# KingOfTheAce2/video-restoration-pipeline-framewright

Hardware: AMD Instinct MI355X
Metric: frames/sec Real-ESRGAN x4 1080p (RRDBNet-x4plus, 1920x1080 -> 7680x4320) (higher is better)
Workload: dtype f16; 1 GPU; RealESRGAN_x4plus x4, 1920x1080 uint8 BGR frames resident in HBM -> 7680x4320 uint8 BGR in HBM, seeded synthetic weights, 43 frames per GPU

## Files before the change

include/framewright_hip.h:

```cpp
#ifndef FRAMEWRIGHT_HIP_H
#define FRAMEWRIGHT_HIP_H

#include <stddef.h>
#include <stdint.h>

#ifdef __cplusplus
extern "C" {
#endif

#define FW_OK 0
#define FW_ERR_INVALID 1
#define FW_ERR_OOM 2
#define FW_ERR_HIP 3
#define FW_ERR_INTERNAL 4

#define FW_HOST 0
#define FW_DEVICE 1

#define FW_DTYPE_BF16 0
#define FW_DTYPE_F16 1

typedef struct fw_rrdbnet fw_rrdbnet;
typedef struct fw_nafnet fw_nafnet;

// ... 35 lines not shown
                    int width, const void* packed_weight, const float* bias, int cout_tiles, int act_lrelu,
                    int upsample2x, const float* res1, float s1, const float* res2, float s2, void* out,
                    int out_cstride, long out_plane_stride, int out_coff, float* out_f32, void* stream);

int fw_conv3x3_nhwc_ex(int dtype, const void* x, int in_cstride, long in_plane_stride, int cin_chunks, int height,
                       int width, const void* packed_weight, const float* bias, int cout_tiles, int act_lrelu,
                       int upsample2x, const float* res1, float s1, const float* res2, float s2, const float* chan_scale,
                       int post_act, int f32_cstride, int f32_coff, void* out, int out_cstride, long out_plane_stride,
                       int out_coff, float* out_f32, void* stream);


int fw_u8_to_nhwc(int dtype, const uint8_t* in_bgr, int height, int width, void* out, int out_cstride, void* stream);

int fw_pixel_shuffle_add_u8(const float* conv, int conv_cstride, const uint8_t* in_bgr, int height, int width, int scale,
                            uint8_t* out_bgr, float* out_rgb_f32, void* stream);

int fw_conv3x3_pair_nhwc(int dtype, const void* x, int in_cstride, long in_plane_stride, int in_chunks, int height,
                         int width, const void* packed_weight_a, const float* bias_a, const void* packed_weight_b,
                         const float* bias_b, void* out_a, void* out_b, int out_cstride, void* stream);

size_t fw_pack_conv_up2x_phase(int dtype, const float* weight, uint16_t* dst);
int fw_conv_up2x_phase_nhwc(int dtype, const void* x, int in_cstride, long in_plane_stride, int height, int width,
                            const void* packed_weight, const float* bias, int act_lrelu, void* out, int out_cstride,
                            long out_plane_stride, void* stream);

size_t fw_pack_conv3x3_wino(int dtype, const float* weight, int cout, int cin, int cin_chunks, uint16_t* dst);
int fw_conv3x3_split_nhwc(int dtype, int winograd, const void* x, int in_cstride, long in_plane_stride, int cin_chunks, int height,
                          int width, const void* packed_weight, const float* bias, float s1, float in_id_scale, int n_id,
                          const long* chunk_off, const float* id_scale, int post_act, void* out, void* out_lo, int out_cstride,
                          long out_plane_stride, int out_coff, void* stream);
int fw_conv3x3_wino_nhwc(int dtype, const void* x, int in_cstride, long in_plane_stride, int cin_chunks, int height, int width,
                         const void* packed_weight, const float* bias, int act_lrelu, void* out, int out_cstride,
                         long out_plane_stride, int out_coff, void* stream);
int fw_conv3x3_wino_check_fields(int* codes, int n);


int fw_nafnet_create(int device_id, int width, int middle_blk_num, const int* enc_blk_nums, const int* dec_blk_nums,
                     int num_levels, int dtype, fw_nafnet** out);

int fw_nafnet_set_tensor(fw_nafnet* net, const char* key, const float* data, size_t numel);
int fw_nafnet_finalize(fw_nafnet* net);

int fw_nafnet_denoise_u8(fw_nafnet* net, const uint8_t* in_bgr, int in_loc, int height, int width, uint8_t* out_bgr,
                         int out_loc, float* out_rgb_f32, void* stream);
double fw_nafnet_flops(const fw_nafnet* net, int height, int width);
int fw_nafnet_destroy(fw_nafnet* net);

#define FW_NAF_PATH_FRONT 1
#define FW_NAF_PATH_TAIL128 2
#define FW_NAF_PATH_TAIL64 4
#define FW_NAF_PATH_GEMM 8
#define FW_NAF_PATH_FUSE_LN 16
int fw_nafnet_run_block(fw_nafnet* net, const char* key, float* stream_f32, int height, int width, float* sca_out, void* stream);
int fw_nafnet_block_paths(fw_nafnet* net, const char* key, int* flags);
int fw_nafnet_run_resample(fw_nafnet* net, int level, int up, const float* src_f32, int height, int width, float* dst_f32, void* stream);
int fw_u8_to_nhwc_padded(int dtype, const uint8_t* in_bgr, int height, int width, int padded_height, int padded_width, void* out,
                         void* stream);


int fw_u8_crop(const uint8_t* src, int height, int width, int y0, int x0, int th, int tw, uint8_t* dst, void* stream);

int fw_tile_blend_accumulate(float* acc, float* wsum, int height, int width, const uint8_t* tile, int y0, int x0, int th,
                             int tw, int overlap, void* stream);

int fw_tile_blend_finish(const float* acc, const float* wsum, int height, int width, uint8_t* out, void* stream);

// ... 222 lines not shown
```

video-restoration-pipeline-framewright_amd/_lib.py:

```python
from __future__ import annotations

import ctypes as C
import threading
from pathlib import Path
from typing import Optional

PKG_DIR = Path(__file__).resolve().parent
LIB_PATH = PKG_DIR / "lib" / "libframewright_hip.so"

FW_OK, FW_ERR_INVALID, FW_ERR_OOM, FW_ERR_HIP, FW_ERR_INTERNAL = 0, 1, 2, 3, 4
FW_HOST, FW_DEVICE = 0, 1
FW_DTYPE_BF16, FW_DTYPE_F16 = 0, 1
FW_NAF_PATH_FRONT, FW_NAF_PATH_TAIL128, FW_NAF_PATH_TAIL64, FW_NAF_PATH_GEMM, FW_NAF_PATH_FUSE_LN = 1, 2, 4, 8, 16
DTYPES = {"bf16": FW_DTYPE_BF16, "bfloat16": FW_DTYPE_BF16, "f16": FW_DTYPE_F16, "fp16": FW_DTYPE_F16,
          "float16": FW_DTYPE_F16, "half": FW_DTYPE_F16}

EXPORTS = [
    "fw_last_error", "fw_abi_version", "fw_device_count",
    "fw_rrdbnet_create", "fw_rrdbnet_set_conv", "fw_rrdbnet_finalize", "fw_rrdbnet_upscale_u8", "fw_rrdbnet_upscale_u16",
    "fw_rrdbnet_workspace_bytes", "fw_rrdbnet_flops", "fw_rrdbnet_profile_enable", "fw_rrdbnet_profile_read",
    "fw_rrdbnet_destroy", "fw_pack_conv3x3", "fw_conv3x3_nhwc",
    "fw_nafnet_create", "fw_nafnet_set_tensor", "fw_nafnet_finalize", "fw_nafnet_denoise_u8", "fw_nafnet_flops",
    "fw_nafnet_destroy", "fw_nafnet_run_block", "fw_nafnet_block_paths", "fw_nafnet_run_resample", "fw_u8_to_nhwc_padded", "fw_u8_crop", "fw_tile_blend_accumulate", "fw_tile_blend_finish", "fw_temporal_average_u8",
    "fw_strength_blend_u8",
    "fw_conv3x3_nhwc_ex", "fw_conv3x3_pair_nhwc", "fw_pack_conv_up2x_phase", "fw_conv_up2x_phase_nhwc", "fw_u8_to_rgb_f32", "fw_resize_bilinear_f32", "fw_ifnet_build_x", "fw_unshuffle2_cast",
    "fw_depth_to_space4_f32", "fw_ifnet_accumulate", "fw_ifnet_blend", "fw_unsharp_mask_u8",
    "fw_ifnet_stage_input", "fw_ifnet_accumulate_d2s", "fw_ifnet_last_flow",
    "fw_ifnet_create", "fw_ifnet_set_tensor", "fw_ifnet_finalize", "fw_ifnet_interp_u8", "fw_ifnet_workspace_bytes", "fw_ifnet_flops",
    "fw_ifnet_destroy",
    "fw_aesrgan_create", "fw_aesrgan_set_tensor", "fw_aesrgan_finalize", "fw_aesrgan_forward_rgb", "fw_aesrgan_workspace_bytes", "fw_aesrgan_destroy",
    "fw_srvgg_create", "fw_srvgg_set_tensor", "fw_srvgg_finalize", "fw_srvgg_upscale_u8", "fw_srvgg_upscale_u16", "fw_resize_lanczos4_u16", "fw_srvgg_workspace_bytes", "fw_srvgg_flops",
    "fw_srvgg_destroy",
    "fw_restormer_create", "fw_restormer_set_tensor", "fw_restormer_finalize", "fw_restormer_denoise_u8",
    "fw_restormer_workspace_bytes", "fw_restormer_destroy", "fw_preserve_edges_scratch_bytes", "fw_preserve_edges_u8",
    "fw_u8_to_nhwc", "fw_pixel_shuffle_add_u8",
    "fw_layernorm_nhwc", "fw_pack_pointwise", "fw_pointwise_nhwc", "fw_dwconv3x3_nhwc", "fw_attn_workspace_floats",
    "fw_attn_matrix", "fw_attn_apply", "fw_attn_pack", "fw_attn_proj_pack", "fw_pixel_shuffle2_f32", "fw_copy_channels_f32", "fw_f32_to_planar", "fw_tap_post_u8",
    "fw_flow_accumulate_u8", "fw_flow_accumulate_finish_u8", "fw_resize_lanczos4_u8", "fw_resize_linear_u8", "fw_face_paste_u8", "fw_grain_addback_u8", "fw_attn_softmax_rows", "fw_pack_pointwise_transposed", "fw_attn_qk_scratch_elems", "fw_attn_matrix_mfma",
    "fw_pack_conv3x3_wino", "fw_conv3x3_split_nhwc", "fw_conv3x3_wino_nhwc", "fw_conv3x3_wino_check_fields",
    "fw_farneback_scratch_bytes", "fw_farneback_flow_u8", "fw_flow_stats_f32", "fw_flow_confidence_f32",
    "fw_nlmeans_scratch_bytes", "fw_nlmeans_u8", "fw_nlmeans_colored_u8", "fw_nlmeans_weight_table", "fw_nlmeans_lab_tables",
    "fw_frame_stats_u8", "fw_flow_accumulate_affine_u8", "fw_add_weighted_u8",
    "fw_bgr_to_lab_u8", "fw_lab_to_bgr_u8", "fw_lab_l_sums_u8", "fw_deflicker_lab_u8", "fw_gamma_lab_tables",
    "fw_scene_ssim_workspace_bytes", "fw_scene_ssim_u8", "fw_hist64x3_u8",
    "fw_pil_lanczos_taps", "fw_pil_thumb_workspace_bytes", "fw_pil_thumb_u8", "fw_dhash_pack_u8",
    "fw_lut3d_apply_u8", "fw_lut3d_apply_u16", "fw_table3_apply_u8",
    "fw_deinterlace_u8", "fw_deinterlace_batch_u8", "fw_interlace_stats_u8", "fw_frame_absdiff_sum_u8",
    "fw_vhs_gray_stats_u8", "fw_vhs_blend_rows_u8", "fw_vhs_rainbow_u8", "fw_vhs_box_gray_sums_u8", "fw_vhs_dropout_repair_u8",
    "fw_vhs_edge_counts_u8", "fw_vhs_chroma_samples_u8", "fw_vhs_chroma_shift_u8", "fw_vhs_column_sums_u8", "fw_vhs_jitter_shifts_u8",
    "fw_vhs_saturation_f64",
]


class FramewrightHipError(RuntimeError):

    def __init__(self, code: int, message: str):
        super().__init__(message)
        self.code = code


class FramewrightOutOfMemory(FramewrightHipError):
    """FW_ERR_OOM — message contains "memory" so reference restorer.py:1746 retries with a smaller tile."""


_lock = threading.Lock()
_lib: Optional[C.CDLL] = None


def _declare(lib: C.CDLL) -> None:
    vp, i32, f32, f64, sz = C.c_void_p, C.c_int, C.c_float, C.c_double, C.c_size_t
    lib.fw_last_error.restype = C.c_char_p
    lib.fw_last_error.argtypes = []
# ... 58 lines not shown
    lib.fw_tile_blend_finish.argtypes = [vp, vp, i32, i32, vp, vp]
    lib.fw_temporal_average_u8.restype = i32
    lib.fw_temporal_average_u8.argtypes = [C.POINTER(vp), C.POINTER(f32), i32, sz, vp, vp]
    lib.fw_strength_blend_u8.restype = i32
    lib.fw_strength_blend_u8.argtypes = [vp, vp, f64, sz, vp, vp]
    lib.fw_grain_addback_u8.restype = i32
    lib.fw_grain_addback_u8.argtypes = [vp, vp, i32, i32, f64, vp, vp, vp]
    lib.fw_resize_lanczos4_u8.restype = i32
    lib.fw_resize_lanczos4_u8.argtypes = [vp, i32, i32, i32, vp, i32, i32, vp]
    lib.fw_resize_linear_u8.restype = i32
    lib.fw_resize_linear_u8.argtypes = [vp, i32, i32, i32, vp, i32, i32, vp]
    lib.fw_face_paste_u8.restype = i32
    lib.fw_face_paste_u8.argtypes = [vp, i32, i32, i32, i32, i32, i32, vp, f64, vp]


def _declare_ifnet(lib: C.CDLL) -> None:
    vp, i32, f32, sz = C.c_void_p, C.c_int, C.c_float, C.c_size_t
    lib.fw_conv3x3_nhwc_ex.restype = i32
    lib.fw_conv3x3_nhwc_ex.argtypes = [i32, vp, i32, C.c_long, i32, i32, i32, vp, vp, i32, i32, i32, vp, f32, vp, f32, vp, i32,
                                       i32, i32, vp, i32, C.c_long, i32, vp, vp]
    lib.fw_pack_conv_up2x_phase.restype = sz
    lib.fw_pack_conv_up2x_phase.argtypes = [i32, vp, vp]
    lib.fw_conv_up2x_phase_nhwc.restype = i32
    lib.fw_conv_up2x_phase_nhwc.argtypes = [i32, vp, i32, C.c_long, i32, i32, vp, vp, i32, vp, i32, C.c_long, vp]
    lib.fw_pack_conv3x3_wino.restype = sz
    lib.fw_pack_conv3x3_wino.argtypes = [i32, vp, i32, i32, i32, vp]
    lib.fw_conv3x3_split_nhwc.restype = i32
    lib.fw_conv3x3_split_nhwc.argtypes = [i32, i32, vp, i32, C.c_long, i32, i32, i32, vp, vp, f32, f32, i32, C.POINTER(C.c_long),
                                          C.POINTER(f32), i32, vp, vp, i32, C.c_long, i32, vp]
    lib.fw_conv3x3_wino_nhwc.restype = i32
    lib.fw_conv3x3_wino_nhwc.argtypes = [i32, vp, i32, C.c_long, i32, i32, i32, vp, vp, i32, vp, i32, C.c_long, i32, vp]
    lib.fw_conv3x3_wino_check_fields.restype = i32
    lib.fw_conv3x3_wino_check_fields.argtypes = [C.POINTER(i32), i32]
    lib.fw_conv3x3_pair_nhwc.restype = i32
    lib.fw_conv3x3_pair_nhwc.argtypes = [i32, vp, i32, C.c_long, i32, i32, i32, vp, vp, vp, vp, vp, vp, i32, vp]
    lib.fw_u8_to_rgb_f32.restype = i32
    lib.fw_u8_to_rgb_f32.argtypes = [vp, i32, i32, i32, i32, vp, vp]
    lib.fw_resize_bilinear_f32.restype = i32
    lib.fw_resize_bilinear_f32.argtypes = [vp, i32, i32, i32, vp, i32, i32, i32, i32, f32, f32, vp]
    lib.fw_ifnet_build_x.restype = i32
    lib.fw_ifnet_build_x.argtypes = [vp, vp, vp, vp, i32, i32, f32, vp, vp]
    lib.fw_unshuffle2_cast.restype = i32
    lib.fw_unshuffle2_cast.argtypes = [i32, vp, i32, i32, i32, i32, i32, vp, i32, vp]
    lib.fw_depth_to_space4_f32.restype = i32
    lib.fw_depth_to_space4_f32.argtypes = [vp, i32, i32, i32, vp, vp]
    lib.fw_ifnet_accumulate.restype = i32
    lib.fw_ifnet_accumulate.argtypes = [vp, i32, i32, i32, i32, f32, vp, vp, i32, vp]
    lib.fw_ifnet_stage_input.restype = i32
    lib.fw_ifnet_stage_input.argtypes = [i32, vp, vp, vp, vp, i32, i32, f32, i32, vp, i32, vp]
    lib.fw_ifnet_accumulate_d2s.restype = i32
    lib.fw_ifnet_accumulate_d2s.argtypes = [vp, i32, i32, i32, i32, i32, f32, vp, vp, i32, vp]
    lib.fw_ifnet_last_flow.restype = i32
    lib.fw_ifnet_last_flow.argtypes = [vp, i32, i32, vp, vp, vp]
    lib.fw_ifnet_blend.restype = i32
    lib.fw_ifnet_blend.argtypes = [vp, vp, vp, vp, i32, i32, i32, i32, vp, vp, vp]
    lib.fw_aesrgan_create.restype = i32
    lib.fw_aesrgan_create.argtypes = [i32, i32, i32, i32, i32, C.POINTER(vp)]
    lib.fw_aesrgan_set_tensor.restype = i32
    lib.fw_aesrgan_set_tensor.argtypes = [vp, C.c_char_p, vp, sz]
    lib.fw_aesrgan_finalize.restype = i32
    lib.fw_aesrgan_finalize.argtypes = [vp]
    lib.fw_aesrgan_forward_rgb.restype = i32
    lib.fw_aesrgan_forward_rgb.argtypes = [vp, vp, i32, i32, vp, vp]
    lib.fw_aesrgan_workspace_bytes.restype = sz
    lib.fw_aesrgan_workspace_bytes.argtypes = [vp, i32, i32]
    lib.fw_aesrgan_destroy.restype = i32
# ... 297 lines not shown
```

video-restoration-pipeline-framewright_amd/csrc/fw_internal.h:

```cpp
#pragma once
#include <hip/hip_runtime.h>
#include <stdint.h>
#include <string.h>
#include <string>
#include <stdexcept>

namespace fw {

enum DType : int { DT_BF16 = 0, DT_F16 = 1 };

enum ConvEpilogue : int {
    EPI_STORE = 0,
    EPI_RESIDUAL = 1,
    EPI_IMAGE = 2,
    EPI_RESIDUAL_SPLIT = 3,
};

struct ConvParams {
    const void* in;
    int in_cstride;
    long in_pstride;
    int cin_chunks;
    int H, W;
    const void* wpk;
// ... 41 lines not shown
    const float* bias_a;
    const void* wpk_b;
    const float* bias_b;
    void* out_a;
    void* out_b;
    int out_cstride;
    const void* zeros;
    unsigned long long* stamps;
};
size_t pack_conv3x3_wino_weights(DType dt, const float* w, int cout, int cin, int cin_chunks, uint16_t* dst);
void launch_conv3x3_wino_split(const ConvParams& p, hipStream_t stream);
void launch_conv3x3_wino_store(const ConvParams& p, hipStream_t stream);
void check_conv3x3_wino(const ConvParams& p, bool split);
void launch_conv3x3_pair(DType dt, const ConvPairParams& p, hipStream_t stream);
const void* conv_zero_page();

struct ConvUpParams {
    const void* in;
    int in_cstride;
    long in_pstride;
    int H, W;
    const void* wpk;
    const float* bias;
    int act;
    void* out;
    int out_cstride;
    long out_pstride;
    const void* zeros;
};
void launch_conv_up2x_phase(DType dt, const ConvUpParams& p, hipStream_t stream);
size_t pack_conv_up2x_phase_weights(DType dt, const float* w, uint16_t* dst);
int conv_num_cus();

void launch_conv3x3(DType dt, int cout_tiles, ConvEpilogue epi, const ConvParams& p, hipStream_t stream);

size_t pack_conv3x3_weights(DType dt, const float* w, int cout, int cin, int cout_tiles, int cin_chunks,
                            uint16_t* dst);

void launch_u8_to_nhwc(DType dt, const uint8_t* in_bgr, int H, int W, void* out, int out_cstride,
                       int unshuffle, hipStream_t stream);
void launch_frame_to_nhwc(DType dt, const void* in_bgr, int bits, int H, int W, void* out, int out_cstride, int unshuffle,
                          hipStream_t stream);
void launch_pixel_shuffle_add(const float* conv, int cstride, const uint8_t* in_bgr, int H, int W, int scale, uint8_t* out_bgr,
                              float* out_rgb, hipStream_t stream);
void launch_pixel_shuffle_add_bits(const float* conv, int cstride, const void* in_bgr, int bits, int H, int W, int scale, void* out_bgr,
                                   float* out_rgb, hipStream_t stream);

enum PointwiseMode : int {
    PW_STORE = 0,
    PW_RESIDUAL = 1,
    PW_GATE = 2,
    PW_SHUFFLE_UP = 3,
};

struct PointwiseParams {
    const void* a;
    int a_f32;
    long lda;
    long M;
    int K;
    int gather2x2;
    int Win;
    int Cin;
    const float* a_scale;
    const float* ln_w;
    const float* ln_b;
// ... 235 lines not shown
```

video-restoration-pipeline-framewright_amd/csrc/rrdbnet.hip:

```cpp
#include <mutex>
#include <vector>
#include <memory>
#include <cstdio>
#include <cstdlib>
#include "engine_common.h"

namespace fw {

struct ConvLayer {
    int cout = 0, cin = 0, ct = 0, chunks = 0;
    void* d_w = nullptr;
    float* d_b = nullptr;
    void* d_wphase = nullptr;
    void* d_wwino = nullptr;
    bool set = false;
};

}

using namespace fw;

namespace fw {
std::string& last_error_ref() {
    thread_local std::string msg;
    return msg;
}
}

struct fw_rrdbnet {
    int device = 0;
    fw::StreamOrder order;
    int num_block = 0;
    int scale = 4;
    DType dt = DT_BF16;
    std::mutex mu;
    ConvLayer conv_first, conv_body, conv_up1, conv_up2, conv_hr, conv_last;
    std::vector<ConvLayer> body;
    DevBuf ws;
    int fuse_mask = 3;
    bool fuse_pairs = true;
    bool split_trunk = true;
    bool rrdb_lo = true;
    int abl_alias = 0;
    bool up_phase = true;
    int c5_wino = 1;
    bool hr_wino = false;
    int abl_rdb3 = 0;
    int graph_mode = 0;
    long graph_max_px = 512L * 512L;
    GraphCache graphs;
    bool warmed = false;
    bool profile = false;
    std::vector<hipEvent_t> ev_pool;
    size_t ev_used = 0;
    double prof_flops = 0;
    hipStream_t prof_stream = nullptr;
};

namespace {

size_t align_up(size_t v, size_t a) { return (v + a - 1) / a * a; }

void trunk_size(const fw_rrdbnet* n, int H, int W, int* Ht, int* Wt) {
    if (n->scale == 2) {
        *Ht = (H + 1) / 2;
        *Wt = (W + 1) / 2;
    } else {
        *Ht = H;
        *Wt = W;
    }
}

struct Plan {
    size_t in_u8, out_u8, in32, cat0, cat1, cat2, F, R, tA, tB, U1, U2, U3, total;
};

Plan make_plan(const fw_rrdbnet* n, int H, int W) {
    int Ht, Wt;
    trunk_size(n, H, W, &Ht, &Wt);
// ... 26 lines not shown
    p.U3 = take(px * 16 * 64 * 2);
    p.total = o;
    return p;
}

ConvLayer* find_layer(fw_rrdbnet* n, const std::string& key, int* want_cout, int* want_cin) {
    const int in_ch = n->scale == 2 ? 12 : 3;
    auto ret = [&](ConvLayer* l, int co, int ci) {
        *want_cout = co;
        *want_cin = ci;
        return l;
    };
    if (key == "conv_first") return ret(&n->conv_first, 64, in_ch);
    if (key == "conv_body") return ret(&n->conv_body, 64, 64);
    if (key == "conv_up1") return ret(&n->conv_up1, 64, 64);
    if (key == "conv_up2") return ret(&n->conv_up2, 64, 64);
    if (key == "conv_hr") return ret(&n->conv_hr, 64, 64);
    if (key == "conv_last") return ret(&n->conv_last, 3, 64);
    int b = -1, r = -1, c = -1;
    char tail = 0;
    if (sscanf(key.c_str(), "body.%d.rdb%d.conv%d%c", &b, &r, &c, &tail) == 3 && b >= 0 && b < n->num_block && r >= 1 &&
        r <= 3 && c >= 1 && c <= 5) {
        ConvLayer* l = &n->body[((size_t)b * 3 + (r - 1)) * 5 + (c - 1)];
        return ret(l, c == 5 ? 64 : 32, 64 + 32 * (c - 1));
    }
    return nullptr;
}

void free_layer(ConvLayer& l) {
    if (l.d_w) (void)hipFree(l.d_w);
    if (l.d_b) (void)hipFree(l.d_b);
    if (l.d_wphase) (void)hipFree(l.d_wphase);
    if (l.d_wwino) (void)hipFree(l.d_wwino);
    l.d_wphase = nullptr;
    l.d_wwino = nullptr;
    l.d_w = nullptr;
    l.d_b = nullptr;
    l.set = false;
}

double conv_flops(const ConvLayer& l, size_t pixels) { return 2.0 * 9.0 * l.cin * l.cout * (double)pixels; }

template <typename F>
void timed(fw_rrdbnet* n, hipStream_t st, double flops, F&& launch) {
    if (!n->profile) {
        launch();
        return;
    }
    if (n->ev_used + 2 > n->ev_pool.size()) {
        size_t old = n->ev_pool.size();
        n->ev_pool.resize(old + 1024);
        for (size_t i = old; i < n->ev_pool.size(); ++i) FW_HIP_CHECK(hipEventCreate(&n->ev_pool[i]));
    }
    FW_HIP_CHECK(hipEventRecord(n->ev_pool[n->ev_used++], st));
    launch();
    FW_HIP_CHECK(hipEventRecord(n->ev_pool[n->ev_used++], st));
    n->prof_flops += flops;
    n->prof_stream = st;
}

void run_conv(fw_rrdbnet* n, const ConvLayer& l, ConvEpilogue epi, ConvParams p, hipStream_t st) {
    p.cin_chunks = l.chunks;
    p.wpk = l.d_w;
    p.bias = l.d_b;
    timed(n, st, conv_flops(l, (size_t)p.H * p.W), [&] { launch_conv3x3(n->dt, l.ct, epi, p, st); });
}
// ... 154 lines not shown
        run_conv(n, n->conv_body, EPI_RESIDUAL, p, st);
        cur = (cur + 1) % ncat;
    }
    auto run_up = [&](const ConvLayer& l, const void* src, long src_pstride, int Hs, int Ws, void* dst, long dst_pstride) {
        if (n->up_phase && l.d_wphase) {
            ConvUpParams u{};
            u.in = src;
            u.in_cstride = 32;
            u.in_pstride = src_pstride;
            u.H = Hs;
            u.W = Ws;
            u.wpk = l.d_wphase;
            u.bias = l.d_b;
            u.act = 1;
            u.out = dst;
            u.out_cstride = 32;
            u.out_pstride = dst_pstride;
            timed(n, st, conv_flops(l, (size_t)4 * Hs * Ws), [&] { launch_conv_up2x_phase(n->dt, u, st); });
        } else {
            ConvParams p = base;
            p.H = 2 * Hs;
            p.W = 2 * Ws;
            p.in = src;
            p.in_pstride = src_pstride;
            p.upsample2x = 1;
            p.out = dst;
            p.out_pstride = dst_pstride;
            p.act = 1;
            run_conv(n, l, EPI_STORE, p, st);
        }
    };
    run_up(n->conv_up1, cat[cur], PL, Ht, Wt, U1, 4 * PL);
    run_up(n->conv_up2, U1, 4 * PL, 2 * Ht, 2 * Wt, U2, 16 * PL);
    {
        ConvParams p = base;
        p.H = 4 * Ht;
        p.W = 4 * Wt;
        p.in = U2;
        p.in_pstride = 16 * PL;
        p.out = U3;
        p.out_pstride = 16 * PL;
        p.act = 1;
        if (n->c5_wino && n->dt == DT_F16 && n->conv_hr.d_wwino && n->hr_wino) {
            p.cin_chunks = n->conv_hr.chunks;
            p.wpk = n->conv_hr.d_wwino;
            p.bias = n->conv_hr.d_b;
            timed(n, st, conv_flops(n->conv_hr, (size_t)p.H * p.W), [&] { launch_conv3x3_wino_store(p, st); });
        } else {
            run_conv(n, n->conv_hr, EPI_STORE, p, st);
        }
    }
    {
        ConvParams p = base;
        p.H = 4 * Ht;
        p.W = 4 * Wt;
        p.in = U3;
        p.in_pstride = 16 * PL;
        if (bits == 16)
            p.out_u16 = (uint16_t*)d_out;
        else
            p.out_u8 = (uint8_t*)d_out;
        p.out_rgb = d_rgb;
        p.img_H = n->scale * H;
        p.img_W = n->scale * W;
        run_conv(n, n->conv_last, EPI_IMAGE, p, st);
    }
}

}

extern "C" {

const char* fw_last_error(void) { return fw::last_error_ref().c_str(); }

int fw_abi_version(void) { return 4; }

int fw_device_count(void) {
    int n = 0;
    if (hipGetDeviceCount(&n) != hipSuccess) return 0;
    return n;
}

int fw_rrdbnet_create(int device_id, int num_block, int scale, int dtype, fw_rrdbnet** out) {
    if (!out) return fail(FW_ERR_INVALID, "fw_rrdbnet_create: out is NULL");
    *out = nullptr;
    if (num_block < 1 || num_block > 64) return fail(FW_ERR_INVALID, "fw_rrdbnet_create: num_block out of range");
    if (scale != 2 && scale != 4) return fail(FW_ERR_INVALID, "fw_rrdbnet_create: scale must be 2 or 4");
    if (dtype != FW_DTYPE_BF16 && dtype != FW_DTYPE_F16) return fail(FW_ERR_INVALID, "fw_rrdbnet_create: bad dtype");
    return guarded([&] {
        int ndev = 0;
        FW_HIP_CHECK(hipGetDeviceCount(&ndev));
        if (device_id < 0 || device_id >= ndev) throw Error(FW_ERR_INVALID, "fw_rrdbnet_create: no such device");
        auto n = std::make_unique<fw_rrdbnet>();
        n->device = device_id;
        n->num_block = num_block;
        n->scale = scale;
        n->dt = (DType)dtype;
        n->body.resize((size_t)num_block * 15);
        if (const char* e = getenv("FW_RRDB_FUSE_PAIRS")) n->fuse_pairs = atoi(e) != 0;
        if (const char* e = getenv("FW_RRDB_FUSE_MASK")) n->fuse_mask = atoi(e) & 3;
        if (const char* e = getenv("FW_RRDB_GRAPH")) n->graph_mode = atoi(e);
        if (const char* e = getenv("FW_RRDB_GRAPH_MAX_PX")) n->graph_max_px = atol(e);
        if (const char* e = getenv("FW_RRDB_SPLIT_TRUNK")) n->split_trunk = atoi(e) != 0;
        if (const char* e = getenv("FW_RRDB_LO")) n->rrdb_lo = atoi(e) != 0;
        if (const char* e = getenv("FW_RRDB_ABL_ALIAS")) n->abl_alias = atoi(e);
        if (const char* e = getenv("FW_RRDB_UP_PHASE")) n->up_phase = atoi(e) != 0;
        if (const char* e = getenv("FW_RRDB_ABL_RDB3")) n->abl_rdb3 = atoi(e);
        if (const char* e = getenv("FW_RRDB_C5_WINO")) n->c5_wino = atoi(e);
        if (const char* e = getenv("FW_RRDB_HR_WINO")) n->hr_wino = atoi(e) != 0;
        *out = n.release();
    });
}

int fw_rrdbnet_set_conv(fw_rrdbnet* n, const char* key, const float* weight, const float* bias, int cout, int cin) {
    if (!n || !key || !weight || !bias) return fail(FW_ERR_INVALID, "fw_rrdbnet_set_conv: NULL argument");
    return guarded([&] {
        std::lock_guard<std::mutex> lk(n->mu);
        int wco = 0, wci = 0;
        ConvLayer* l = find_layer(n, key, &wco, &wci);
        if (!l) throw Error(FW_ERR_INVALID, std::string("fw_rrdbnet_set_conv: unknown key '") + key + "'");
        if (cout != wco || cin != wci)
            throw Error(FW_ERR_INVALID, std::string("fw_rrdbnet_set_conv: shape mismatch for '") + key + "': got [" +
                                            std::to_string(cout) + "," + std::to_string(cin) + ",3,3], expected [" +
                                            std::to_string(wco) + "," + std::to_string(wci) + ",3,3]");
        DevGuard dg(n->device);
        free_layer(*l);
        l->cout = cout;
        l->cin = cin;
        l->ct = (cout + 31) / 32;
        l->chunks = (cin + 31) / 32;
        const size_t ne = pack_conv3x3_weights(n->dt, nullptr, cout, cin, l->ct, l->chunks, nullptr);
        std::vector<uint16_t> packed(ne);
        pack_conv3x3_weights(n->dt, weight, cout, cin, l->ct, l->chunks, packed.data());
        std::vector<float> b(32 * l->ct, 0.f);
        for (int i = 0; i < cout; ++i) b[i] = bias[i];
        FW_HIP_CHECK(hipMalloc(&l->d_w, ne * 2));
        FW_HIP_CHECK(hipMalloc((void**)&l->d_b, b.size() * 4));
        FW_HIP_CHECK(hipMemcpy(l->d_w, packed.data(), ne * 2, hipMemcpyHostToDevice));
        FW_HIP_CHECK(hipMemcpy(l->d_b, b.data(), b.size() * 4, hipMemcpyHostToDevice));
        if (n->dt == DT_F16 && cout == 64 && (cin == 192 || l == &n->conv_hr)) {
            const size_t nw = pack_conv3x3_wino_weights(n->dt, nullptr, cout, cin, l->chunks, nullptr);
            std::vector<uint16_t> wn(nw);
            pack_conv3x3_wino_weights(n->dt, weight, cout, cin, l->chunks, wn.data());
            FW_HIP_CHECK(hipMalloc(&l->d_wwino, nw * 2));
            FW_HIP_CHECK(hipMemcpy(l->d_wwino, wn.data(), nw * 2, hipMemcpyHostToDevice));
        }
        if (l == &n->conv_up1 || l == &n->conv_up2) {
            const size_t np = pack_conv_up2x_phase_weights(n->dt, nullptr, nullptr);
            std::vector<uint16_t> ph(np);
            pack_conv_up2x_phase_weights(n->dt, weight, ph.data());
            FW_HIP_CHECK(hipMalloc(&l->d_wphase, np * 2));
            FW_HIP_CHECK(hipMemcpy(l->d_wphase, ph.data(), np * 2, hipMemcpyHostToDevice));
        }
        l->set = true;
    });
}

int fw_rrdbnet_finalize(fw_rrdbnet* n) {
    if (!n) return fail(FW_ERR_INVALID, "fw_rrdbnet_finalize: NULL");
    std::lock_guard<std::mutex> lk(n->mu);
    const ConvLayer* singles[] = {&n->conv_first, &n->conv_body, &n->conv_up1, &n->conv_up2, &n->conv_hr, &n->conv_last};
    const char* names[] = {"conv_first", "conv_body", "conv_up1", "conv_up2", "conv_hr", "conv_last"};
    for (int i = 0; i < 6; ++i)
        if (!singles[i]->set) return fail(FW_ERR_INVALID, std::string("fw_rrdbnet_finalize: missing ") + names[i]);
    for (size_t i = 0; i < n->body.size(); ++i)
        if (!n->body[i].set)
            return fail(FW_ERR_INVALID, "fw_rrdbnet_finalize: missing body." + std::to_string(i / 15) + ".rdb" +
                                            std::to_string((i / 5) % 3 + 1) + ".conv" + std::to_string(i % 5 + 1));
    return FW_OK;
}

size_t fw_rrdbnet_workspace_bytes(const fw_rrdbnet* n, int H, int W) {
    if (!n || H < 1 || W < 1) return 0;
    return make_plan(n, H, W).total;
}

double fw_rrdbnet_flops(const fw_rrdbnet* n, int H, int W) {
    if (!n || H < 1 || W < 1) return 0.0;
    int Ht, Wt;
// ... 212 lines not shown
    if (dtype != FW_DTYPE_BF16 && dtype != FW_DTYPE_F16) return fail(FW_ERR_INVALID, "fw_conv3x3_split_nhwc: bad dtype");
    if (winograd != 0 && winograd != 1) return fail(FW_ERR_INVALID, "fw_conv3x3_split_nhwc: winograd must be 0 or 1");
    if (winograd && dtype != FW_DTYPE_F16) return fail(FW_ERR_INVALID, "fw_conv3x3_split_nhwc: the Winograd form is f16 only");
    if (n_id < 0 || n_id > 6) return fail(FW_ERR_INVALID, "fw_conv3x3_split_nhwc: n_id must be in [0, 6]");
    if (n_id > 0 && (!chunk_off || !id_scale)) return fail(FW_ERR_INVALID, "fw_conv3x3_split_nhwc: residual planes need chunk_off and id_scale");
    return guarded([&] {
        ConvParams p{};
        p.in = x;
        p.in_cstride = in_cstride;
        p.in_pstride = in_plane_stride > 0 ? in_plane_stride : 32;
        p.cin_chunks = cin_chunks;
        p.H = H;
        p.W = W;
        p.wpk = packed_weight;
        p.bias = bias;
        p.s1 = s1;
        p.s2 = 1.f;
        p.in_id_scale = in_id_scale;
        p.n_id = n_id;
        for (int i = 0; i < n_id; ++i) {
            p.chunk_off[i] = chunk_off[i];
            p.id_scale[i] = id_scale[i];
        }
        p.post_act = post_act;
        p.out = out;
        p.out_lo = out_lo;
        p.out_cstride = out_cstride;
        p.out_pstride = out_plane_stride > 0 ? out_plane_stride : 32;
        p.out_coff = out_coff;
        if (winograd)
            launch_conv3x3_wino_split(p, (hipStream_t)stream);
        else
            launch_conv3x3((DType)dtype, 2, EPI_RESIDUAL_SPLIT, p, (hipStream_t)stream);
    });
}

int fw_conv3x3_wino_nhwc(int dtype, const void* x, int in_cstride, long in_plane_stride, int cin_chunks, int H, int W,
                         const void* packed_weight, const float* bias, int act_lrelu, void* out, int out_cstride, long out_plane_stride,
                         int out_coff, void* stream) {
    if (!x || !packed_weight || !bias || !out) return fail(FW_ERR_INVALID, "fw_conv3x3_wino_nhwc: NULL argument");
    if (dtype != FW_DTYPE_F16) return fail(FW_ERR_INVALID, "fw_conv3x3_wino_nhwc: the Winograd form is f16 only");
    if (act_lrelu != 0 && act_lrelu != 1) return fail(FW_ERR_INVALID, "fw_conv3x3_wino_nhwc: act_lrelu must be 0 or 1");
    return guarded([&] {
        ConvParams p{};
        p.in = x;
        p.in_cstride = in_cstride;
        p.in_pstride = in_plane_stride > 0 ? in_plane_stride : 32;
        p.cin_chunks = cin_chunks;
        p.H = H;
        p.W = W;
        p.wpk = packed_weight;
        p.bias = bias;
        p.act = act_lrelu;
        p.out = out;
        p.out_cstride = out_cstride;
        p.out_pstride = out_plane_stride > 0 ? out_plane_stride : 32;
        p.out_coff = out_coff;
        launch_conv3x3_wino_store(p, (hipStream_t)stream);
    });
}

int fw_conv3x3_wino_check_fields(int* codes, int n) {
    static const float one = 1.f;
    static char dummy[16];
    ConvParams ok{};
    ok.H = ok.W = 16;
// ... 95 lines not shown
```

Baseline: 14.72 frames/s.

## Fuse conv_hr and conv_last into one kernel writing the final image

Adds a kernel that runs conv_hr (64->64 3x3 with LeakyReLU) and then, in its epilogue, applies conv_last (64->3 3x3) to the activated tile held in registers. conv_last is done as three per-column MFMA pointwise products combined through lane permutes, an LDS exchange, and a carried row halo between vertically adjacent tiles. It writes u8/u16/f32 output directly. This removes the write and re-read of the full-resolution 64-channel U3 tensor and one launch at 7680x4320. The cost is an extra epilogue per tile, overlapping tiles (30-wide outputs from 32-wide tiles), and band-ordered tiles that recompute one tile to obtain the carry. It is enabled by default when the tile count is large, unless the Winograd conv_hr path is selected.

```diff
diff --git a/include/framewright_hip.h b/include/framewright_hip.h
--- a/include/framewright_hip.h
+++ b/include/framewright_hip.h
@@ -91,6 +91,11 @@
 int fw_conv3x3_wino_nhwc(int dtype, const void* x, int in_cstride, long in_plane_stride, int cin_chunks, int height, int width,
                          const void* packed_weight, const float* bias, int act_lrelu, void* out, int out_cstride,
                          long out_plane_stride, int out_coff, void* stream);
+size_t fw_pack_conv_last_pointwise(int dtype, const float* weight, uint16_t* dst);
+int fw_conv3x3_hr_last_nhwc(int dtype, int fused, const void* x, int in_cstride, long in_plane_stride, int height, int width,
+                            const void* packed_w_hr, const float* bias_hr, const void* packed_w_last, const void* packed_w_last_pw,
+                            const float* bias_last, void* scratch_u3, int img_height, int img_width, uint8_t* out_u8,
+                            uint16_t* out_u16, float* out_rgb_f32, void* stream);
 int fw_conv3x3_wino_check_fields(int* codes, int n);
 
 
diff --git a/video-restoration-pipeline-framewright_amd/_lib.py b/video-restoration-pipeline-framewright_amd/_lib.py
--- a/video-restoration-pipeline-framewright_amd/_lib.py
+++ b/video-restoration-pipeline-framewright_amd/_lib.py
@@ -38,6 +38,7 @@
     "fw_attn_matrix", "fw_attn_apply", "fw_attn_pack", "fw_attn_proj_pack", "fw_pixel_shuffle2_f32", "fw_copy_channels_f32", "fw_f32_to_planar", "fw_tap_post_u8",
     "fw_flow_accumulate_u8", "fw_flow_accumulate_finish_u8", "fw_resize_lanczos4_u8", "fw_resize_linear_u8", "fw_face_paste_u8", "fw_grain_addback_u8", "fw_attn_softmax_rows", "fw_pack_pointwise_transposed", "fw_attn_qk_scratch_elems", "fw_attn_matrix_mfma",
     "fw_pack_conv3x3_wino", "fw_conv3x3_split_nhwc", "fw_conv3x3_wino_nhwc", "fw_conv3x3_wino_check_fields",
+    "fw_pack_conv_last_pointwise", "fw_conv3x3_hr_last_nhwc",
     "fw_farneback_scratch_bytes", "fw_farneback_flow_u8", "fw_flow_stats_f32", "fw_flow_confidence_f32",
     "fw_nlmeans_scratch_bytes", "fw_nlmeans_u8", "fw_nlmeans_colored_u8", "fw_nlmeans_weight_table", "fw_nlmeans_lab_tables",
     "fw_frame_stats_u8", "fw_flow_accumulate_affine_u8", "fw_add_weighted_u8",
@@ -162,6 +163,10 @@
     lib.fw_conv3x3_wino_nhwc.argtypes = [i32, vp, i32, C.c_long, i32, i32, i32, vp, vp, i32, vp, i32, C.c_long, i32, vp]
     lib.fw_conv3x3_wino_check_fields.restype = i32
     lib.fw_conv3x3_wino_check_fields.argtypes = [C.POINTER(i32), i32]
+    lib.fw_pack_conv_last_pointwise.restype = sz
+    lib.fw_pack_conv_last_pointwise.argtypes = [i32, vp, vp]
+    lib.fw_conv3x3_hr_last_nhwc.restype = i32
+    lib.fw_conv3x3_hr_last_nhwc.argtypes = [i32, i32, vp, i32, C.c_long, i32, i32, vp, vp, vp, vp, vp, vp, i32, i32, vp, vp, vp, vp]
     lib.fw_conv3x3_pair_nhwc.restype = i32
     lib.fw_conv3x3_pair_nhwc.argtypes = [i32, vp, i32, C.c_long, i32, i32, i32, vp, vp, vp, vp, vp, vp, i32, vp]
     lib.fw_u8_to_rgb_f32.restype = i32
diff --git a/video-restoration-pipeline-framewright_amd/csrc/conv3x3_hr_last.hip b/video-restoration-pipeline-framewright_amd/csrc/conv3x3_hr_last.hip
--- /dev/null
+++ b/video-restoration-pipeline-framewright_amd/csrc/conv3x3_hr_last.hip
@@ -0,0 +1,335 @@
+#include "fw_internal.h"
+#include "conv_common.h"
+
+#ifndef FW_DMA_SLOT_W
+#define FW_DMA_SLOT_W 2
+#define FW_DMA_SLOT_A 6
+#endif
+
+namespace fw {
+
+constexpr int HL_TW = TILE_W - 2;
+constexpr int HL_FRAGS = 6;
+
+struct HrLastParams {
+    ConvParams p;
+    const void* wlast;
+    const float* blast;
+};
+
+struct HrLastSmem {
+    using SM = Smem<2>;
+    static constexpr int FRAG = SM::TOTAL;
+    static constexpr int CARRY = FRAG + HL_FRAGS * 64;
+    static constexpr int BIAS = CARRY + 3 * TILE_W;
+    static constexpr int TOTAL = BIAS + 17;
+};
+static_assert(HrLastSmem::TOTAL * 16 <= 160 * 1024, "LDS");
+static_assert(3 * TILE_H * TILE_W <= ACT_REGION, "the exchange of r fits an activation stage");
+static_assert(NWAVES == 8 && RPW == 2, "written for 8 waves of 2 rows");
+
+__device__ __forceinline__ float lane_read(int addr4, float v) {
+    return __builtin_bit_cast(float, __builtin_amdgcn_ds_bpermute(addr4, __builtin_bit_cast(int, v)));
+}
+
+__device__ __forceinline__ f32x4 lrelu4_builtin(f32x4 v) {
+    const f32x4 t = v * 0.2f;
+    f32x4 o;
+#pragma unroll
+    for (int j = 0; j < 4; ++j) o[j] = __builtin_fmaxf(v[j], t[j]);
+    return o;
+}
+
+template <typename T>
+__global__ __launch_bounds__(64 * NWAVES, WAVES_PER_SIMD) void conv3x3_hr_last_kernel(const HrLastParams hp) {
+    const ConvParams& p = hp.p;
+    using SM = Smem<2>;
+    using HS = HrLastSmem;
+    __shared__ __attribute__((aligned(16))) uint4 lds[HS::TOTAL];
+    constexpr int NA = SM::NA;
+    constexpr int NW = 4;
+    static_assert(NA == 2, "the exchange scratch relies on two activation stages");
+
+    const int tid = threadIdx.x;
+    const int wave = __builtin_amdgcn_readfirstlane(tid >> 6);
+    const int lane = tid & 63;
+    const int q = lane & 15;
+    const int sl = lane >> 4;
+
+    const TileBand band;
+    const int tiles_x = (p.W + HL_TW - 1) / HL_TW;
+    const int tiles_y = (p.H + TILE_H) / TILE_H;
+    const int ntiles = tiles_x * tiles_y;
+    int t_lo, t_hi;
+    band.range(ntiles, &t_lo, &t_hi);
+    if (t_lo >= t_hi) return;
+    const int t_first = t_lo - ((t_lo % tiles_y) != 0 ? 1 : 0);
+    const int nch = p.cin_chunks;
+    const int nitems = (t_hi - t_first) * nch;
+    auto origin = [&](int t, int* y0, int* x0) {
+        const int tx = t / tiles_y, ty = t - tx * tiles_y;
+        *y0 = ty * TILE_H;
+        *x0 = tx * HL_TW - 1;
+    };
+
+    float* bias_l = reinterpret_cast<float*>(lds + HS::BIAS);
+    if (tid < HL_FRAGS * 64) lds[HS::FRAG + tid] = reinterpret_cast<const uint4*>(hp.wlast)[tid];
+    if (tid < 64) bias_l[tid] = p.bias[tid];
+    if (tid >= 64 && tid < 68) bias_l[tid] = tid < 67 ? hp.blast[tid - 64] : 0.f;
+    __syncthreads();
+
+    unsigned relb[ACT_ITERS];
+#pragma unroll
+    for (int i = 0; i < ACT_ITERS; ++i) {
+        const HaloPiece h = halo_piece((ACT_ITERS * wave + i) * 64 + lane);
+        relb[i] = (unsigned)(((h.row * p.W + h.px) * p.in_cstride + h.s * 8) * 2) + (unsigned)(4 - i % 5) * 1024u;
+    }
+    const unsigned lds_base = (unsigned)(size_t)(lds_ptr_t)lds;
+    const char* in = reinterpret_cast<const char*>(p.in);
+    const char* w_b = reinterpret_cast<const char*>(p.wpk);
+    const unsigned lane16 = lane * 16;
+    const long chunk_bytes = p.in_pstride * 2;
+
+    unsigned a_ok = 0;
+    bool a_all = true;
+    const char* a_src = nullptr;
+    int a_n = 0, a_t = t_first, a_c = 0;
+    auto plan_tile = [&]() {
+        int ty0, tx0;
+        origin(a_t, &ty0, &tx0);
+        a_src = in + ((long)(ty0 - 1) * p.W + (tx0 - 1)) * p.in_cstride * 2;
+        a_ok = 0;
+#pragma unroll
+        for (int i = 0; i < ACT_ITERS; ++i) {
+            const int idx = (ACT_ITERS * wave + i) * 64 + lane;
+            const HaloPiece h = halo_piece(idx);
+            const int gy = ty0 - 1 + h.row;
+            const int gx = tx0 - 1 + h.px;
+            if (idx < ACT_PIECES && (unsigned)gy < (unsigned)p.H && (unsigned)gx < (unsigned)p.W) a_ok |= 1u << i;
+        }
+        a_all = __builtin_amdgcn_readfirstlane(__all(a_ok == (1u << ACT_ITERS) - 1u)) != 0;
+    };
+    auto issue_act = [&]() {
+        if (a_c == 0) plan_tile();
+        const unsigned dst = (unsigned)((a_n % NA) * ACT_REGION + ACT_ITERS * wave * 64);
+        if (a_all) {
+#pragma unroll
+            for (int bt = 0; bt < ACT_ITERS / 5; ++bt) glds16_batch_a(a_src, relb + 5 * bt, lds_base + (dst + (5 * bt + 4) * 64) * 16u);
+        } else {
+#pragma unroll
+            for (int i = 0; i < ACT_ITERS; ++i)
+                glds16_v(((a_ok >> i) & 1u) ? a_src + (relb[i] - (unsigned)(4 - i % 5) * 1024u) : reinterpret_cast<const char*>(p.zeros),
+                         lds_base + (dst + i * 64) * 16u);
+        }
+        ++a_n;
+        if (++a_c == nch) {
+            a_c = 0;
+            ++a_t;
+        } else {
+            a_src += chunk_bytes;
+        }
+    };
+    auto issue_w = [&](int c, int ws) {
+        const int half = wave / (NWAVES / 2), k = wave % (NWAVES / 2);
+        issue_w_half(w_b + (size_t)c * (W_FRAGS * 2 * 1024) + W_FRAGS * half * 1024,
+                     lds_base + (unsigned)(SM::W_BASE + ws * SM::W_REGION + W_FRAGS * half * 64) * 16u, k, lane16);
+    };
+
+    int rd_off[3][2];
+#pragma unroll
+    for (int dx = 0; dx < 3; ++dx)
+#pragma unroll
+        for (int ph = 0; ph < 2; ++ph) rd_off[dx][ph] = halo_rd_off(RPW * wave, 16 * ph + q + dx, sl);
+
+    const int lane_l = ((lane & 48) | ((q + 15) & 15)) * 4;
+    const int lane_r = ((lane & 48) | ((q + 1) & 15)) * 4;
+
+    f32x4 acc[RPW][NW][2];
+
+    issue_w(0, 0);
+    issue_act();
+
+    float4* carry = reinterpret_cast<float4*>(lds + HS::CARRY);
+    const uint4* frag = lds + HS::FRAG + lane;
+
+    int n = 0;
+    for (int t = t_first; t < t_hi; ++t) {
+        int y0, x0;
+        origin(t, &y0, &x0);
+#pragma unroll
+        for (int w = 0; w < NW; ++w) {
+            const f32x4 bv = *reinterpret_cast<const f32x4*>(bias_l + 16 * w + 4 * sl);
+#pragma unroll
+            for (int row = 0; row < RPW; ++row)
+#pragma unroll
+                for (int ph = 0; ph < 2; ++ph) acc[row][w][ph] = bv;
+        }
+
+        for (int c = 0; c < nch; ++c, ++n) {
+            if (c > 0 || t == t_first) FW_WAIT_VMCNT(0);
+            __syncthreads();
+            const bool do_w = n + 1 < nitems;
+            const bool do_a = n + NA - 1 < nitems;
+            const int c1 = (c + 1 == nch) ? 0 : c + 1;
+            auto dma_slot = [&](int d) {
+                if (d == FW_DMA_SLOT_W) {
+                    if (do_w) issue_w(c1, (n + 1) & 1);
+                } else if (d == FW_DMA_SLOT_A) {
+                    if (do_a) issue_act();
+                }
+            };
+            const uint4* a = lds + (n % NA) * ACT_REGION;
+            const uint4* wl = lds + SM::W_BASE + (n & 1) * SM::W_REGION + lane;
+            auto& slot_fn = dma_slot;
+            conv_item<T, NW, 0>(
+                acc, a, wl, rd_off, [](int tap, int w) { return tap * NW + w; }, slot_fn, [](const uint4 (&)[RPW][2]) {}, [](int) {});
+        }
+
+        FW_WAIT_VMCNT(0);
+        const bool interior = x0 >= 0 && x0 + TILE_W <= p.W && y0 + TILE_H <= p.H;
+        f32x4 r[RPW][2];
+#pragma unroll
+        for (int row = 0; row < RPW; ++row) {
+            f32x4 z[3][2];
+#pragma unroll
+            for (int ph = 0; ph < 2; ++ph) {
+                uint4 hk[2];
+#pragma unroll
+                for (int c2 = 0; c2 < 2; ++c2) {
+                    hk[c2] = pair16<T>(lrelu4_builtin(acc[row][2 * c2][ph]), lrelu4_builtin(acc[row][2 * c2 + 1][ph]));
+                    if (!interior && !(y0 + RPW * wave + row < p.H && (unsigned)(x0 + 16 * ph + q) < (unsigned)p.W))
+                        hk[c2] = make_uint4(0, 0, 0, 0);
+                }
+#pragma unroll
+                for (int dx = 0; dx < 3; ++dx) {
+                    f32x4 zz = {0.f, 0.f, 0.f, 0.f};
+                    zz = Op<T>::mfma16(frag[(2 * dx) * 64], hk[0], zz);
+                    zz = Op<T>::mfma16(frag[(2 * dx + 1) * 64], hk[1], zz);
+                    z[dx][ph] = zz;
+                }
+            }
+#pragma unroll
+            for (int j = 0; j < 3; ++j) {
+                float zl[2], zr[2];
+#pragma unroll
+                for (int ph = 0; ph < 2; ++ph) {
+                    zl[ph] = lane_read(lane_l, z[0][ph][j]);
+                    zr[ph] = lane_read(lane_r, z[2][ph][j]);
+                }
+                r[row][0][j] = (zl[0] + z[1][0][j]) + (q == 15 ? zr[1] : zr[0]);
+                r[row][1][j] = ((q == 0 ? zl[0] : zl[1]) + z[1][1][j]) + zr[1];
+            }
+            r[row][0][3] = 0.f;
+            r[row][1][3] = 0.f;
+        }
+        __syncthreads();
+        float4* S = reinterpret_cast<float4*>(lds + ((n - 1) % NA) * ACT_REGION);
+        if (sl < 3) {
+#pragma unroll
+            for (int row = 0; row < RPW; ++row)
+#pragma unroll
+                for (int ph = 0; ph < 2; ++ph)
+                    S[(sl * TILE_H + RPW * wave + row) * TILE_W + 16 * ph + q] =
+                        make_float4(r[row][ph][0], r[row][ph][1], r[row][ph][2], 0.f);
+        }
+        __syncthreads();
+        {
+            const int o = RPW * wave + (lane >> 5), cp = lane & 31;
+            const bool col_top = y0 == 0;
+            const float4 zero4 = make_float4(0.f, 0.f, 0.f, 0.f);
+            float4 a0, a1;
+            if (wave == 0) {
+                const float4 c0 = carry[(o == 0 ? 0 : 2) * TILE_W + cp];
+                const float4 c1 = o == 0 ? carry[TILE_W + cp] : S[(TILE_H + 0) * TILE_W + cp];
+                a0 = col_top ? zero4 : c0;
+                a1 = (col_top && o == 0) ? zero4 : c1;
+            } else {
+                a0 = S[(o - 2) * TILE_W + cp];
+                a1 = S[(TILE_H + o - 1) * TILE_W + cp];
+            }
+            const float4 a2 = S[(2 * TILE_H + o) * TILE_W + cp];
+            if (wave == 0) {
+                carry[lane] = S[(lane < 32 ? 14 : TILE_H + 15) * TILE_W + cp];
+                if (lane < 32) carry[2 * TILE_W + cp] = S[15 * TILE_W + cp];
+            }
+            const float cr = ((bias_l[64] + a0.x) + a1.x) + a2.x;
+            const float cg = ((bias_l[65] + a0.y) + a1.y) + a2.y;
+            const float cb = ((bias_l[66] + a0.z) + a1.z) + a2.z;
+            const int y = y0 - 1 + o, x = x0 + cp;
+            if (t >= t_lo && cp >= 1 && cp <= HL_TW && y >= 0 && y < p.H && x < p.W && y < p.img_H && x < p.img_W) {
+                const size_t pix = (size_t)y * p.img_W + x;
+                if (p.out_rgb) {
+                    float* op = p.out_rgb + pix * 3;
+                    op[0] = cr;
+                    op[1] = cg;
+                    op[2] = cb;
+                }
+                if (p.out_u16) {
+                    uint16_t* op = p.out_u16 + pix * 3;
+                    op[0] = (uint16_t)rintf(fminf(fmaxf(cb, 0.f), 1.f) * 65535.f);
+                    op[1] = (uint16_t)rintf(fminf(fmaxf(cg, 0.f), 1.f) * 65535.f);
+                    op[2] = (uint16_t)rintf(fminf(fmaxf(cr, 0.f), 1.f) * 65535.f);
+                }
+                if (p.out_u8) {
+                    uint8_t* op = p.out_u8 + pix * 3;
+                    op[0] = (uint8_t)rintf(fminf(fmaxf(cb, 0.f), 1.f) * 255.f);
+                    op[1] = (uint8_t)rintf(fminf(fmaxf(cg, 0.f), 1.f) * 255.f);
+                    op[2] = (uint8_t)rintf(fminf(fmaxf(cr, 0.f), 1.f) * 255.f);
+                }
+            }
+        }
+    }
+}
+
+bool hr_last_default(int H, int W) {
+    const long tiles = (long)((W + HL_TW - 1) / HL_TW) * ((H + TILE_H) / TILE_H);
+    return tiles >= 6L * conv_num_cus();
+}
+
+void launch_conv3x3_hr_last(DType dt, const ConvParams& hr, const void* wlast, const float* bias_last, hipStream_t stream) {
+    HrLastParams hp{};
+    hp.p = hr;
+    hp.p.zeros = conv_zero_page();
+    hp.wlast = wlast;
+    hp.blast = bias_last;
+    const ConvParams& p = hp.p;
+    if (p.H <= 0 || p.W <= 0) throw Error(1, "conv3x3_hr_last: empty problem");
+    if (p.cin_chunks != 2) throw Error(1, "conv3x3_hr_last: conv_hr contracts 64 channels");
+    if (!p.in || !p.wpk || !p.bias || !wlast || !bias_last) throw Error(1, "conv3x3_hr_last: NULL argument");
+    if (p.upsample2x || p.n_groups > 1 || p.out_f32 || p.res1 || p.res2 || p.out_lo || p.chan_scale)
+        throw Error(1, "conv3x3_hr_last: unsupported conv_hr field");
+    if (p.in_cstride < 32 || (p.in_cstride & 7) || p.in_pstride < 32 || (p.in_pstride & 7) ||
+        (p.in_pstride == 32 && p.in_cstride < 64 && (long)p.H * p.W > 1))
+        throw Error(1, "conv3x3_hr_last: bad input channel/plane stride");
+    if (p.img_H <= 0 || p.img_W <= 0 || p.img_H > p.H || p.img_W > p.W) throw Error(1, "conv3x3_hr_last: bad image size");
+    if (!p.out_u8 && !p.out_u16 && !p.out_rgb) throw Error(1, "conv3x3_hr_last: no output");
+    const int tiles = ((p.W + HL_TW - 1) / HL_TW) * ((p.H + TILE_H) / TILE_H);
+    const int ncu = conv_num_cus();
+    dim3 grid(tiles < ncu ? tiles : ncu), block(64 * NWAVES);
+    if (dt == DT_BF16)
+        hipLaunchKernelGGL(conv3x3_hr_last_kernel<__bf16>, grid, block, 0, stream, hp);
+    else
+        hipLaunchKernelGGL(conv3x3_hr_last_kernel<_Float16>, grid, block, 0, stream, hp);
+    FW_HIP_CHECK(hipGetLastError());
+}
+
+size_t pack_conv_last_pointwise(DType dt, const float* w, uint16_t* dst) {
+    const size_t n = (size_t)HL_FRAGS * 64 * 8;
+    if (!dst) return n;
+    size_t o = 0;
+    for (int dx = 0; dx < 3; ++dx)
+        for (int c2 = 0; c2 < 2; ++c2)
+            for (int lane = 0; lane < 64; ++lane)
+                for (int j = 0; j < 8; ++j) {
+                    const int row = lane & 15, s = lane >> 4;
+                    const int dy = row >> 2, c = row & 3;
+                    const int ls = (s & 1) ? 2 + (s >> 1) : (s >> 1);
+                    const int ch = 32 * c2 + 8 * ls + j;
+                    float val = 0.f;
+                    if (dy < 3 && c < 3) val = w[((size_t)c * 64 + ch) * 9 + dy * 3 + dx];
+                    dst[o++] = f32_to_operand(dt, val);
+                }
+    return n;
+}
+
+}
diff --git a/video-restoration-pipeline-framewright_amd/csrc/fw_internal.h b/video-restoration-pipeline-framewright_amd/csrc/fw_internal.h
--- a/video-restoration-pipeline-framewright_amd/csrc/fw_internal.h
+++ b/video-restoration-pipeline-framewright_amd/csrc/fw_internal.h
@@ -97,6 +97,10 @@
 size_t pack_conv_up2x_phase_weights(DType dt, const float* w, uint16_t* dst);
 int conv_num_cus();
 
+void launch_conv3x3_hr_last(DType dt, const ConvParams& hr, const void* wlast, const float* bias_last, hipStream_t stream);
+size_t pack_conv_last_pointwise(DType dt, const float* w, uint16_t* dst);
+bool hr_last_default(int H, int W);
+
 void launch_conv3x3(DType dt, int cout_tiles, ConvEpilogue epi, const ConvParams& p, hipStream_t stream);
 
 size_t pack_conv3x3_weights(DType dt, const float* w, int cout, int cin, int cout_tiles, int cin_chunks,
diff --git a/video-restoration-pipeline-framewright_amd/csrc/rrdbnet.hip b/video-restoration-pipeline-framewright_amd/csrc/rrdbnet.hip
--- a/video-restoration-pipeline-framewright_amd/csrc/rrdbnet.hip
+++ b/video-restoration-pipeline-framewright_amd/csrc/rrdbnet.hip
@@ -13,6 +13,7 @@
     float* d_b = nullptr;
     void* d_wphase = nullptr;
     void* d_wwino = nullptr;
+    void* d_wlast = nullptr;
     bool set = false;
 };
 
@@ -45,6 +46,7 @@
     bool up_phase = true;
     int c5_wino = 1;
     bool hr_wino = false;
+    int hr_last = -1;
     int abl_rdb3 = 0;
     int graph_mode = 0;
     long graph_max_px = 512L * 512L;
@@ -137,6 +139,8 @@
     if (l.d_b) (void)hipFree(l.d_b);
     if (l.d_wphase) (void)hipFree(l.d_wphase);
     if (l.d_wwino) (void)hipFree(l.d_wwino);
+    if (l.d_wlast) (void)hipFree(l.d_wlast);
+    l.d_wlast = nullptr;
     l.d_wphase = nullptr;
     l.d_wwino = nullptr;
     l.d_w = nullptr;
@@ -357,16 +361,43 @@
     };
     run_up(n->conv_up1, cat[cur], PL, Ht, Wt, U1, 4 * PL);
     run_up(n->conv_up2, U1, 4 * PL, 2 * Ht, 2 * Wt, U2, 16 * PL);
+    ConvParams hr = base;
+    hr.H = 4 * Ht;
+    hr.W = 4 * Wt;
+    hr.in = U2;
+    hr.in_pstride = 16 * PL;
+    ConvParams img = base;
+    img.H = 4 * Ht;
+    img.W = 4 * Wt;
+    if (bits == 16)
+        img.out_u16 = (uint16_t*)d_out;
+    else
+        img.out_u8 = (uint8_t*)d_out;
+    img.out_rgb = d_rgb;
+    img.img_H = n->scale * H;
+    img.img_W = n->scale * W;
+    const bool hr_wino = n->c5_wino && n->dt == DT_F16 && n->conv_hr.d_wwino && n->hr_wino;
+    if (!hr_wino && (n->hr_last < 0 ? hr_last_default(hr.H, hr.W) : n->hr_last != 0)) {
+        ConvParams p = hr;
+        p.out_u8 = img.out_u8;
+        p.out_u16 = img.out_u16;
+        p.out_rgb = img.out_rgb;
+        p.img_H = img.img_H;
+        p.img_W = img.img_W;
+        p.cin_chunks = n->conv_hr.chunks;
+        p.wpk = n->conv_hr.d_w;
+        p.bias = n->conv_hr.d_b;
+        const size_t px = (size_t)p.H * p.W;
+        timed(n, st, conv_flops(n->conv_hr, px) + conv_flops(n->conv_last, px),
+              [&] { launch_conv3x3_hr_last(n->dt, p, n->conv_last.d_wlast, n->conv_last.d_b, st); });
+        return;
+    }
     {
-        ConvParams p = base;
-        p.H = 4 * Ht;
-        p.W = 4 * Wt;
-        p.in = U2;
-        p.in_pstride = 16 * PL;
+        ConvParams p = hr;
         p.out = U3;
         p.out_pstride = 16 * PL;
         p.act = 1;
-        if (n->c5_wino && n->dt == DT_F16 && n->conv_hr.d_wwino && n->hr_wino) {
+        if (hr_wino) {
             p.cin_chunks = n->conv_hr.chunks;
             p.wpk = n->conv_hr.d_wwino;
             p.bias = n->conv_hr.d_b;
@@ -376,18 +407,9 @@
         }
     }
     {
-        ConvParams p = base;
-        p.H = 4 * Ht;
-        p.W = 4 * Wt;
+        ConvParams p = img;
         p.in = U3;
         p.in_pstride = 16 * PL;
-        if (bits == 16)
-            p.out_u16 = (uint16_t*)d_out;
-        else
-            p.out_u8 = (uint8_t*)d_out;
-        p.out_rgb = d_rgb;
-        p.img_H = n->scale * H;
-        p.img_W = n->scale * W;
         run_conv(n, n->conv_last, EPI_IMAGE, p, st);
     }
 }
@@ -433,6 +455,7 @@
         if (const char* e = getenv("FW_RRDB_ABL_RDB3")) n->abl_rdb3 = atoi(e);
         if (const char* e = getenv("FW_RRDB_C5_WINO")) n->c5_wino = atoi(e);
         if (const char* e = getenv("FW_RRDB_HR_WINO")) n->hr_wino = atoi(e) != 0;
+        if (const char* e = getenv("FW_RRDB_HR_LAST")) n->hr_last = atoi(e) != 0;
         *out = n.release();
     });
 }
@@ -470,6 +493,12 @@
             FW_HIP_CHECK(hipMalloc(&l->d_wwino, nw * 2));
             FW_HIP_CHECK(hipMemcpy(l->d_wwino, wn.data(), nw * 2, hipMemcpyHostToDevice));
         }
+        if (l == &n->conv_last) {
+            std::vector<uint16_t> pw(pack_conv_last_pointwise(n->dt, nullptr, nullptr));
+            pack_conv_last_pointwise(n->dt, weight, pw.data());
+            FW_HIP_CHECK(hipMalloc(&l->d_wlast, pw.size() * 2));
+            FW_HIP_CHECK(hipMemcpy(l->d_wlast, pw.data(), pw.size() * 2, hipMemcpyHostToDevice));
+        }
         if (l == &n->conv_up1 || l == &n->conv_up2) {
             const size_t np = pack_conv_up2x_phase_weights(n->dt, nullptr, nullptr);
             std::vector<uint16_t> ph(np);
@@ -748,6 +777,68 @@
             launch_conv3x3_wino_split(p, (hipStream_t)stream);
         else
             launch_conv3x3((DType)dtype, 2, EPI_RESIDUAL_SPLIT, p, (hipStream_t)stream);
+    });
+}
+
+size_t fw_pack_conv_last_pointwise(int dtype, const float* weight, uint16_t* dst) {
+    if (dtype != FW_DTYPE_BF16 && dtype != FW_DTYPE_F16) return 0;
+    if (dst && !weight) return 0;
+    return pack_conv_last_pointwise((DType)dtype, weight, dst);
+}
+
+int fw_conv3x3_hr_last_nhwc(int dtype, int fused, const void* x, int in_cstride, long in_plane_stride, int H, int W,
+                            const void* packed_w_hr, const float* bias_hr, const void* packed_w_last, const void* packed_w_last_pw,
+                            const float* bias_last, void* scratch_u3, int img_H, int img_W, uint8_t* out_u8, uint16_t* out_u16,
+                            float* out_rgb_f32, void* stream) {
+    if (!x || !packed_w_hr || !bias_hr || !bias_last) return fail(FW_ERR_INVALID, "fw_conv3x3_hr_last_nhwc: NULL argument");
+    if (dtype != FW_DTYPE_BF16 && dtype != FW_DTYPE_F16) return fail(FW_ERR_INVALID, "fw_conv3x3_hr_last_nhwc: bad dtype");
+    if (fused != 0 && fused != 1) return fail(FW_ERR_INVALID, "fw_conv3x3_hr_last_nhwc: fused must be 0 or 1");
+    if (fused ? !packed_w_last_pw : (!packed_w_last || !scratch_u3))
+        return fail(FW_ERR_INVALID, "fw_conv3x3_hr_last_nhwc: missing conv_last weights or scratch for this form");
+    if (H < 1 || W < 1 || img_H < 1 || img_W < 1 || img_H > H || img_W > W) return fail(FW_ERR_INVALID, "fw_conv3x3_hr_last_nhwc: bad size");
+    if (!out_u8 && !out_u16 && !out_rgb_f32) return fail(FW_ERR_INVALID, "fw_conv3x3_hr_last_nhwc: no output");
+    return guarded([&] {
+        ConvParams hr{};
+        hr.in = x;
+        hr.in_cstride = in_cstride;
+        hr.in_pstride = in_plane_stride > 0 ? in_plane_stride : 32;
+        hr.cin_chunks = 2;
+        hr.H = H;
+        hr.W = W;
+        hr.wpk = packed_w_hr;
+        hr.bias = bias_hr;
+        hr.s1 = hr.s2 = 1.f;
+        ConvParams img{};
+        img.H = H;
+        img.W = W;
+        img.s1 = img.s2 = 1.f;
+        img.out_u8 = out_u8;
+        img.out_u16 = out_u16;
+        img.out_rgb = out_rgb_f32;
+        img.img_H = img_H;
+        img.img_W = img_W;
+        if (fused) {
+            hr.out_u8 = out_u8;
+            hr.out_u16 = out_u16;
+            hr.out_rgb = out_rgb_f32;
+            hr.img_H = img_H;
+            hr.img_W = img_W;
+            launch_conv3x3_hr_last((DType)dtype, hr, packed_w_last_pw, bias_last, (hipStream_t)stream);
+            return;
+        }
+        const long plane = (long)H * W * 32;
+        hr.out = scratch_u3;
+        hr.out_cstride = 32;
+        hr.out_pstride = plane;
+        hr.act = 1;
+        launch_conv3x3((DType)dtype, 2, EPI_STORE, hr, (hipStream_t)stream);
+        img.in = scratch_u3;
+        img.in_cstride = 32;
+        img.in_pstride = plane;
+        img.cin_chunks = 2;
+        img.wpk = packed_w_last;
+        img.bias = bias_last;
+        launch_conv3x3((DType)dtype, 1, EPI_IMAGE, img, (hipStream_t)stream);
     });
 }
 
```

Result: faster. 14.96 frames/s (median of 6 runs) (+1.6%).
